# XiandaGuo/OpenStereo

Hardware: NVIDIA H100
Metric: stereo_pairs_per_sec_gwcnet_256x512_d192 (higher is better)
Workload: dtype f32

## Files before the change

### include/openstereo_b200.h

```cpp
#ifndef OPENSTEREO_B200_H_
#define OPENSTEREO_B200_H_

#include <stddef.h>
#include <stdint.h>

#ifdef __cplusplus
extern "C" {
#endif

#define OSB_OK 0
#define OSB_EINVAL 1
#define OSB_ECUDA 2
#define OSB_EUNSUPPORTED 3

#define OSB_ACT_NONE 0
#define OSB_ACT_RELU 1
#define OSB_ACT_LEAKY 2
#define OSB_ACT_RELU6 3
#define OSB_ACT_SIGMOID 4
#define OSB_ACT_TANH 5

typedef void* osb_stream_t;

int osb_abi_version(void);
const char* osb_last_error(void);
uint64_t osb_launch_count(void);
int osb_tc_overflow_count(osb_stream_t stream, int reset, unsigned int* count);
int osb_tc_overflow_poll(osb_stream_t stream, unsigned int* host_pinned);
const unsigned int* osb_tc_overflow_flag(void);
float osb_set_rz_kappa(float kappa);
int osb_set_persistent_grid_cap(int cap);
const char* osb_tc_last_variant(void);
const char* osb_volume_last_variant(void);


int osb_gwc_volume_fwd(const float* ref, const float* tgt, float* out, int B, int C, int H, int W,
                       int D, int G, osb_stream_t stream);

int osb_concat_volume_fwd(const float* ref, const float* tgt, float* out, int B, int C, int H,
                          int W, int D, int mask_left, osb_stream_t stream);

int osb_gwc_concat_volume_fwd(const float* ref_gwc, const float* tgt_gwc, const float* ref_cat,
                              const float* tgt_cat, float* out, int B, int Cg, int Cc, int H, int W,
                              int D, int G, osb_stream_t stream);

int osb_corr_volume_fwd(const float* left, const float* right, float* out, int B, int C, int H,
                        int W, int D, osb_stream_t stream);


int osb_softargmin_fwd(const float* cost, float* out, int B, int D, int H, int W, float alpha,
                       float start, float step, int normalize, osb_stream_t stream);

int osb_upsample_softargmin_fwd(const float* cost, float* out, int B, int Dl, int Hl, int Wl, int D,
                                int H, int W, int align_corners, osb_stream_t stream);

int osb_upsample_softargmin_values_fwd(const float* cost, const float* values, float* out, int B, int Dl, int Hl, int Wl,
                                       int D, int H, int W, int align_corners, osb_stream_t stream);

int osb_epe_partial_fwd(const float* pred, const float* gt, float* out, int B, int HW, float maxdisp,
                        osb_stream_t stream);


int osb_conv3d_k3_bn_act_fwd(const float* x, const float* w_packed, const float* scale,
                             const float* shift, const float* residual, const float* gate, float* y,
                             int B, int Cin, int Cout, int D, int H, int W, int stride, int act,
                             osb_stream_t stream);

// ... 114 lines not shown
```

### openstereo_b200/_lib.py

```python
import ctypes
import os

_PKG = os.path.dirname(os.path.abspath(__file__))
LIB_PATH = os.path.join(_PKG, "lib", "libopenstereo_b200.so")

_f32p = ctypes.c_void_p
_i = ctypes.c_int
_f = ctypes.c_float
_s = ctypes.c_void_p

SIGNATURES = {
    "osb_gwc_volume_fwd": [_f32p, _f32p, _f32p, _i, _i, _i, _i, _i, _i, _s],
    "osb_concat_volume_fwd": [_f32p, _f32p, _f32p, _i, _i, _i, _i, _i, _i, _s],
    "osb_gwc_concat_volume_fwd": [_f32p, _f32p, _f32p, _f32p, _f32p, _i, _i, _i, _i, _i, _i, _i, _s],
    "osb_corr_volume_fwd": [_f32p, _f32p, _f32p, _i, _i, _i, _i, _i, _s],
    "osb_softargmin_fwd": [_f32p, _f32p, _i, _i, _i, _i, _f, _f, _f, _i, _s],
    "osb_upsample_softargmin_fwd": [_f32p, _f32p, _i, _i, _i, _i, _i, _i, _i, _i, _s],
    "osb_epe_partial_fwd": [_f32p, _f32p, _f32p, _i, _i, _f, _s],
    "osb_conv3d_k3_bn_act_fwd": [_f32p] * 7 + [_i] * 8 + [_s],
    "osb_deconv3d_bn_act_fwd": [_f32p] * 6 + [_i] * 8 + [_s],
    "osb_conv3d_1x1_bn_act_fwd": [_f32p, _f32p, _i] + [_f32p] * 6 + [_i] * 8 + [_s],
    "osb_conv3d_tc_supported": [_i, _i, _i, _i],
    "osb_conv3d_tc_kc": [_i, _i, _i, _i],
    "osb_tc_general_width": [_i],
    "osb_conv3d_s2_tc_supported": [_i, _i, _i, _i, _i],
    "osb_deconv3d_tc_supported": [_i, _i, _i],
    "osb_deconv3d_k3_tc_fwd": [_f32p] * 6 + [_i] * 9 + [_s],
    "osb_conv3d_k3_s2_tc_fwd": [_f32p] * 6 + [_i] * 9 + [_s],
    "osb_conv3d_k3_tc_fwd": [_f32p] * 6 + [_i] * 9 + [_s],
    "osb_conv3d_k3_tc_ncdhw_fwd": [_f32p] * 6 + [_i] * 9 + [_s],
    "osb_conv3d_k3_tc_split_fwd": [_f32p] * 6 + [_i] * 10 + [_s],
    "osb_ncdhw_to_split": [_f32p, _f32p] + [_i] * 5 + [_s],
    "osb_conv3d_k3_tc_gate_fwd": [_f32p] * 7 + [_i] * 7 + [_s],
    "osb_deconv3d_k4_tc_supported": [_i, _i, _i],
    "osb_conv3d_k3_tc_cs_fwd": [_f32p] * 7 + [_i] * 8 + [_s],
    "osb_conv3d_k3_s2_tc_cs_fwd": [_f32p] * 5 + [_i] * 8 + [_s],
    "osb_deconv3d_k4_tc_cs_fwd": [_f32p] * 5 + [_i] * 8 + [_s],
# ... 87 lines not shown
```

### openstereo_b200/aggregation.py

```python
import torch

from . import ops
from .ops import ACT_LEAKY, ACT_NONE, ACT_RELU, ACT_RELU6


class _Packed:
    __slots__ = ("w", "scale", "shift", "stride", "kernel", "transposed", "cin", "cout", "_w5", "_tc")

    def __init__(self, conv, bn=None):
        self._tc = {}
        self._w5 = conv.weight.detach() if conv.weight.dim() == 5 else None
        self.cin, self.cout = (conv.in_channels, conv.out_channels)
        self.transposed = isinstance(conv, (torch.nn.ConvTranspose3d, torch.nn.ConvTranspose2d))
        self.kernel = int(conv.kernel_size[0])
        self.stride = int(conv.stride[0])
        self._validate(conv)
        wt = conv.weight
        if wt.dim() == 4:
            wt = wt.unsqueeze(2)
        if self.transposed:
            self.w = ops.pack_deconv_weight(wt)
        else:
            self.w = ops.pack_conv_weight(wt)
        if self.kernel == 1:
# ... 41 lines not shown
    kc = ops.conv3d_tc_kc(layer.cin, layer.cout, width)
    if not kc:
        return None
    if kc not in layer._tc:
        layer._tc[kc] = ops.pack_tc_weight(layer._w5, kc, pad_cout_to=16 if layer.cout < 16 else None)
    return layer._tc[kc]


def _tc_ok(layer, width):
    return _tc_weight(layer, width) is not None


def _conv_tc(layer, x_ndhwc, act=ACT_NONE, residual=None, out_ndhwc=True, res_ndhwc=True, in_ncdhw=False, out_split=False):
    wt = _tc_weight(layer, x_ndhwc.shape[4] if in_ncdhw else x_ndhwc.shape[3])
    return ops.conv3d_k3_tc(x_ndhwc, wt, layer.scale, layer.shift, residual, act, out_ndhwc, res_ndhwc, in_ncdhw,
                            out_split=out_split)


def _split_chain_ok(width, *layers):
    return USE_TENSOR_CORES and all(ops.conv3d_tc_kc(l.cin, l.cout, width) == 32 for l in layers)


def _stem_in(layer, volume, act, out_split=False):
    if ops.conv3d_tc_kc(layer.cin, layer.cout, volume.shape[-1]) == 32:
        return _conv_tc(layer, volume, act, in_ncdhw=True, out_split=out_split)
    return _conv_tc(layer, ops.to_ndhwc(volume), act)


def _conv_auto(layer, x, act=ACT_NONE, residual=None):
    if layer.stride == 1 and _tc_ok(layer, x.shape[-1]):
        return _conv_tc(layer, ops.to_ndhwc(x), act, residual, out_ndhwc=False, res_ndhwc=False)
    if (USE_TENSOR_CORES and layer.stride == 2 and layer.kernel == 3 and not layer.transposed and layer._w5 is not None
            and ops.conv3d_s2_tc_supported(layer.cin, layer.cout, x.shape[2], x.shape[3], x.shape[4])):
        if "s2" not in layer._tc:
            layer._tc["s2"] = ops.pack_tc_weight(layer._w5, 16, kw_order=(1, 0, 2))
        return ops.conv3d_k3_s2_tc(ops.to_ndhwc(x), layer._tc["s2"], layer.scale, layer.shift, residual, act)
    return _conv(layer, x, act, residual)


def _deconv(layer, x, act=ACT_NONE, residual=None):
    if (USE_TENSOR_CORES and layer.transposed and layer.kernel == 3 and layer._w5 is not None
            and ops.deconv3d_tc_supported(layer.cin, layer.cout, x.shape[-1])):
        if "dc" not in layer._tc:
            layer._tc["dc"] = ops.pack_tc_deconv_weight(layer._w5)
        return ops.deconv3d_k3_tc(ops.to_ndhwc(x), layer._tc["dc"], layer.scale, layer.shift, residual, act)
    return ops.deconv3d(x, layer.w, layer.scale, layer.shift, residual, layer.kernel, act)
# ... 88 lines not shown
    head0, cls = classif3
    width = out.shape[3]
    if _tc_ok(cls, width):
        mid = _conv_tc(head0, out, ACT_RELU, out_split=_split_chain_ok(width, head0, cls))
        return _conv_tc(cls, mid, ACT_NONE, out_ndhwc=False, res_ndhwc=False)
    if cls.cin == 32 and cls.cout == 1 and cls._w5 is not None and cls.stride == 1:
        if "c1" not in cls._tc:
            cls._tc["c1"] = ops.pack_c1_weight(cls._w5)
        head = _conv_tc(head0, out, ACT_RELU)
        return ops.conv3d_k3_c1_ndhwc(head, cls._tc["c1"], cls.scale, cls.shift)
    head = _conv_tc(head0, out, ACT_RELU, out_ndhwc=False)
    return _conv(cls, head)


class GwcAggregation(_Engine):

    def _pack(self):
        m = self.module
        self.dres0 = [_Packed(m.dres0[0][0], m.dres0[0][1]), _Packed(m.dres0[2][0], m.dres0[2][1])]
        self.dres1 = [_Packed(m.dres1[0][0], m.dres1[0][1]), _Packed(m.dres1[2][0], m.dres1[2][1])]
        self.hg = [_GwcHourglass(m.dres2), _GwcHourglass(m.dres3), _GwcHourglass(m.dres4)]
        self.classif3 = [_Packed(m.classif3[0][0], m.classif3[0][1]), _Packed(m.classif3[2])]

    def logits(self, volume):
        volume = self._check(volume)
        self._ensure(volume.device)
        width = volume.shape[-1]
        stem_tc = all(_tc_ok(l, width) for l in (self.dres0[0], self.dres0[1], self.dres1[0], self.dres1[1]))
        b, _, dd, hh, ww = volume.shape
        if stem_tc and _tc_ok(self.classif3[0], width) and all(_hg_channels_last_ok(hg, (b, dd, hh, ww, 32)) for hg in self.hg):
            split = _split_chain_ok(width, self.dres0[0], self.dres0[1], self.dres1[0], self.dres1[1])
            c = _conv_tc(self.dres0[1], _stem_in(self.dres0[0], volume, ACT_RELU, out_split=split), ACT_RELU, out_split=split)
            out = _conv_tc(self.dres1[1], _conv_tc(self.dres1[0], c, ACT_RELU, out_split=split), ACT_NONE, residual=c)
            for hg in self.hg:
                out = _gwc_hourglass_channels_last(hg, out)
            return _classif3_channels_last(self.classif3, out)
        if stem_tc:
            c = _conv_tc(self.dres0[1], _stem_in(self.dres0[0], volume, ACT_RELU), ACT_RELU)
            cost0 = _conv_tc(self.dres1[1], _conv_tc(self.dres1[0], c, ACT_RELU), ACT_NONE, residual=c, out_ndhwc=False)
        else:
            c = _conv(self.dres0[1], _conv(self.dres0[0], volume, ACT_RELU), ACT_RELU)
            cost0 = _conv(self.dres1[1], _conv(self.dres1[0], c, ACT_RELU), ACT_NONE, residual=c)
        out = cost0
        for hg in self.hg:
            out = hg(out)
        if _tc_ok(self.classif3[0], width):
            head = _conv_tc(self.classif3[0], ops.to_ndhwc(out), ACT_RELU, out_ndhwc=False)
        else:
            head = _conv(self.classif3[0], out, ACT_RELU)
        return _conv(self.classif3[1], head)

    def __call__(self, volume, h, w):
        mon = self._watch(volume.device)
        out = ops.upsample_softargmin(self.logits(volume), self.module.maxdisp, h, w, align_corners=False)
        if mon is not None:
            mon.poll()
        return out


class CascadeAggregation(GwcAggregation):

    def __call__(self, cost, fine_d, fine_h, fine_w, disp_range_samples):
        mon = self._watch(cost.device)
        assert tuple(disp_range_samples.shape[1:]) == (fine_d, fine_h, fine_w)
        out = ops.upsample_softargmin_values(self.logits(cost), disp_range_samples, align_corners=False)
        if mon is not None:
            mon.poll()
        return out


class _PSMHourglass:
    def __init__(self, m):
        self.conv1, self.conv2 = _Packed(m.conv1[0], m.conv1[1]), _Packed(m.conv2[0], m.conv2[1])
        self.conv3, self.conv4 = _Packed(m.conv3[0], m.conv3[1]), _Packed(m.conv4[0], m.conv4[1])
        self.conv5, self.conv6 = _Packed(m.conv5[0], m.conv5[1]), _Packed(m.conv6[0], m.conv6[1])

    def __call__(self, x, presqu, postsqu, skip):
# ... 630 lines not shown
```

### openstereo_b200/csrc/volume.cu

```cuda
#include <cstdlib>

#include "common.cuh"

namespace osb {

constexpr int kTileW = 128;
constexpr int kChunkD = 64;
constexpr int kRowW = kTileW + kChunkD;
constexpr int kJG = 4;

struct VolParams {
  const float* ref_g;
  const float* tgt_g;
  const float* ref_c;
  const float* tgt_c;
  float* out;
  int B, Cg, Cc, H, W, D, G, K;
  int Ctot, oc_cat;
  int GU, n_gwc_units, n_cat_units, w_tiles, d_chunks;
  int mask_left, use_tma, vec_ok;
  int order;
  float inv_k;
};

__device__ __forceinline__ float4 load_quad(const float* row, int w, int W, bool vec) {
  if (vec && w + 3 < W) return __ldg(reinterpret_cast<const float4*>(row + w));
  float4 v;
  v.x = (w + 0 < W) ? __ldg(row + w + 0) : 0.f;
  v.y = (w + 1 < W) ? __ldg(row + w + 1) : 0.f;
  v.z = (w + 2 < W) ? __ldg(row + w + 2) : 0.f;
  v.w = (w + 3 < W) ? __ldg(row + w + 3) : 0.f;
  return v;
}

__device__ __forceinline__ void store_quad(float* row, int w, int W, bool vec, float4 v) {
  if (vec && w + 3 < W) {
    st_cs_f4(row + w, v);
  } else {
    if (w + 0 < W) __stcs(row + w + 0, v.x);
    if (w + 1 < W) __stcs(row + w + 1, v.y);
    if (w + 2 < W) __stcs(row + w + 2, v.z);
    if (w + 3 < W) __stcs(row + w + 3, v.w);
  }
}

struct Item {
  int unit, h, b, w0, d0;
};
__device__ __forceinline__ Item decode_item(const VolParams& p, int it) {
  Item i;
  const int units = p.n_gwc_units + p.n_cat_units;
  if (p.order == 1) {
    i.h = it % p.H;
    it /= p.H;
    i.unit = it % units;
    it /= units;
  } else {
    i.unit = it % units;
    it /= units;
    i.h = it % p.H;
    it /= p.H;
  }
  i.d0 = (it % p.d_chunks) * kChunkD;
  it /= p.d_chunks;
  i.w0 = (it % p.w_tiles) * kTileW;
  i.b = it / p.w_tiles;
  return i;
}

template <bool VEC, bool K4>
__global__ void __launch_bounds__(256, 2) volume_kernel(const __grid_constant__ CUtensorMap tgt_map, const VolParams p,
                                                        const int total_items) {
  extern __shared__ __align__(128) float smem[];
  const int warp = threadIdx.x >> 5, lane = threadIdx.x & 31;
  const int rows = p.n_gwc_units > 0 ? p.GU * p.K : p.GU;
  const size_t buf_floats = (size_t)rows * kRowW;
  uint64_t* bars = reinterpret_cast<uint64_t*>(smem + 2 * buf_floats);
  const size_t HW = (size_t)p.H * p.W;
  constexpr bool vec = VEC;
  const uint32_t tx_bytes = (uint32_t)rows * kRowW * 4u;

  if (p.use_tma && threadIdx.x == 0) {
    tma_prefetch_desc(&tgt_map);
    mbar_init(&bars[0], 1);
    mbar_init(&bars[1], 1);
    fence_mbar_init();
  }
  __syncthreads();

  auto issue_tma = [&](int it, int stage) {
    const Item n = decode_item(p, it);
    if (n.unit < p.n_gwc_units) {
      fence_proxy_async();
      mbar_arrive_expect_tx(&bars[stage], tx_bytes);
      tma_load_3d(smem + stage * buf_floats, &tgt_map, &bars[stage], n.w0 - n.d0 - kChunkD, n.h,
                  n.b * p.Cg + n.unit * p.GU * p.K);
    }
  };

  int stage = 0;
  uint32_t phase0 = 0, phase1 = 0;
  if (p.use_tma && threadIdx.x == 0 && (int)blockIdx.x < total_items) issue_tma(blockIdx.x, 0);

// ... 10 lines not shown

    if (cur.unit < p.n_gwc_units) {
      const int g0 = cur.unit * p.GU;
      if (p.use_tma) {
        if (stage == 0) {
          mbar_wait(&bars[0], phase0);
          phase0 ^= 1;
        } else {
          mbar_wait(&bars[1], phase1);
          phase1 ^= 1;
        }
      } else {
        const int live = min(rows, p.Cg - g0 * p.K);
        for (int idx = threadIdx.x; idx < live * kRowW; idx += blockDim.x) {
          const int r = idx / kRowW, c = idx - r * kRowW;
          const int gw = col0 + c;
          float v = 0.f;
          if (gw >= 0 && gw < p.W) v = __ldg(p.tgt_g + ((size_t)(b * p.Cg + g0 * p.K + r) * p.H + h) * p.W + gw);
          buf[idx] = v;
        }
        __syncthreads();
      }
      const int g = g0 + warp;
      if (g < p.G && wq < p.W) {
        const float* lrow = p.ref_g + ((size_t)(b * p.Cg + g * p.K) * p.H + h) * p.W;
        const float* rbase = buf + (size_t)warp * p.K * kRowW;
        float* obase = p.out + (((size_t)(b * p.Ctot + g) * p.D) * p.H + h) * p.W;
        for (int j0 = 0; j0 < nquads; j0 += kJG) {
          float acc[kJG][4][4];
#pragma unroll
          for (int jj = 0; jj < kJG; ++jj)
#pragma unroll
            for (int i = 0; i < 4; ++i)
#pragma unroll
              for (int a = 0; a < 4; ++a) acc[jj][i][a] = 0.f;
          const int win = kChunkD + 4 * (lane - j0) - 16;
          for (int k0 = 0; k0 < p.K; k0 += 4) {
            float4 lq[4];
#pragma unroll
            for (int kk = 0; kk < 4; ++kk)
              lq[kk] = (K4 || k0 + kk < p.K) ? load_quad(lrow + (size_t)(k0 + kk) * HW, wq, p.W, vec) : make_float4(0.f, 0.f, 0.f, 0.f);
#pragma unroll
            for (int kk = 0; kk < 4; ++kk) {
              if (K4 || k0 + kk < p.K) {
                const float l[4] = {lq[kk].x * p.inv_k, lq[kk].y * p.inv_k, lq[kk].z * p.inv_k, lq[kk].w * p.inv_k};
                float r[20];
                const float4* rp = reinterpret_cast<const float4*>(rbase + (size_t)(k0 + kk) * kRowW + win);
#pragma unroll
                for (int n = 0; n < 5; ++n) {
                  const float4 t = rp[n];
                  r[4 * n + 0] = t.x, r[4 * n + 1] = t.y, r[4 * n + 2] = t.z, r[4 * n + 3] = t.w;
                }
#pragma unroll
                for (int jj = 0; jj < kJG; ++jj)
#pragma unroll
                  for (int i = 0; i < 4; ++i)
#pragma unroll
                    for (int a = 0; a < 4; ++a) acc[jj][i][a] = fmaf(l[a], r[16 - 4 * jj + a - i], acc[jj][i][a]);
              }
            }
          }
#pragma unroll
          for (int jj = 0; jj < kJG; ++jj) {
#pragma unroll
            for (int i = 0; i < 4; ++i) {
              const int d = d0 + 4 * (j0 + jj) + i;
              if (4 * (j0 + jj) + i < nd) {
                float4 v;
                v.x = (wq + 0 >= d) ? acc[jj][i][0] : 0.f;
                v.y = (wq + 1 >= d) ? acc[jj][i][1] : 0.f;
                v.z = (wq + 2 >= d) ? acc[jj][i][2] : 0.f;
                v.w = (wq + 3 >= d) ? acc[jj][i][3] : 0.f;
                store_quad(obase + (size_t)d * HW, wq, p.W, vec, v);
              }
            }
          }
        }
      }
    } else {
      const int oc = (cur.unit - p.n_gwc_units) * p.GU + warp;
      if (oc < 2 * p.Cc) {
        const bool left = oc < p.Cc;
        float* obase = p.out + (((size_t)(b * p.Ctot + p.oc_cat + oc) * p.D) * p.H + h) * p.W;
        if (left) {
          if (wq < p.W) {
            const float4 v = load_quad(p.ref_c + ((size_t)(b * p.Cc + oc) * p.H + h) * p.W, wq, p.W, vec);
            for (int dd = 0; dd < nd; ++dd) {
              const int d = d0 + dd;
              float4 o = v;
              if (p.mask_left) {
                o.x = (wq + 0 >= d) ? v.x : 0.f;
                o.y = (wq + 1 >= d) ? v.y : 0.f;
                o.z = (wq + 2 >= d) ? v.z : 0.f;
                o.w = (wq + 3 >= d) ? v.w : 0.f;
              }
              store_quad(obase + (size_t)d * HW, wq, p.W, vec, o);
            }
          }
        } else {
          float* row = buf + (size_t)warp * kRowW;
          const float* src = p.tgt_c + ((size_t)(b * p.Cc + (oc - p.Cc)) * p.H + h) * p.W;
          for (int c = lane; c < kRowW; c += 32) {
            const int gw = col0 + c;
            row[c] = (gw >= 0 && gw < p.W) ? __ldg(src + gw) : 0.f;
          }
          __syncwarp();
          if (wq < p.W) {
            for (int j = 0; j < nquads; ++j) {
              const float4 lo = *reinterpret_cast<const float4*>(row + kChunkD + 4 * (lane - j) - 4);
              const float4 hi = *reinterpret_cast<const float4*>(row + kChunkD + 4 * (lane - j));
              const float wv[8] = {lo.x, lo.y, lo.z, lo.w, hi.x, hi.y, hi.z, hi.w};
#pragma unroll
              for (int i = 0; i < 4; ++i) {
                const int d = d0 + 4 * j + i;
                if (4 * j + i < nd) {
                  float4 o;
                  o.x = wv[4 - i], o.y = wv[5 - i], o.z = wv[6 - i], o.w = wv[7 - i];
                  store_quad(obase + (size_t)d * HW, wq, p.W, vec, o);
                }
              }
            }
          }
        }
      }
    }
    __syncthreads();
  }
}

static thread_local const char* g_volume_variant = "";

static int launch_volume(const float* ref_g, const float* tgt_g, const float* ref_c, const float* tgt_c, float* out,
                         int B, int Cg, int Cc, int H, int W, int D, int G, int mask_left, cudaStream_t stream, int reduce_sum = 0) {
  OSB_REQUIRE(B > 0 && H > 0 && W > 0 && D > 0, "volume: empty shape B=%d H=%d W=%d D=%d", B, H, W, D);
  OSB_REQUIRE(Cg >= 0 && Cc >= 0 && (Cg > 0 || Cc > 0), "volume: no channels");
  int K = 0;
  if (Cg > 0) {
    OSB_REQUIRE(G > 0 && Cg % G == 0, "groupwise_correlation: C=%d not divisible by num_groups=%d", Cg, G);
    K = Cg / G;
    OSB_REQUIRE(K <= 144, "volume: %d channels per group exceeds the 144 supported (two-stage 192-float rows in 227 KB)", K);
  } else {
    G = 0;
  }
  VolParams p{};
  p.ref_g = ref_g, p.tgt_g = tgt_g, p.ref_c = ref_c, p.tgt_c = tgt_c, p.out = out;
  p.B = B, p.Cg = Cg, p.Cc = Cc, p.H = H, p.W = W, p.D = D, p.G = G, p.K = K;
  p.Ctot = G + 2 * Cc, p.oc_cat = G;
  int GU = 8;
  if (Cg > 0) {
    GU = G < 8 ? G : 8;
    while (GU > 1 && GU * K > 128) GU >>= 1;
  }
  p.GU = GU;
  p.n_gwc_units = Cg > 0 ? (G + GU - 1) / GU : 0;
  p.n_cat_units = Cc > 0 ? (2 * Cc + GU - 1) / GU : 0;
  p.w_tiles = (W + kTileW - 1) / kTileW;
  p.d_chunks = (D + kChunkD - 1) / kChunkD;
  p.mask_left = mask_left;
  {
    static const int order = [] {
      const char* e = getenv("OSB_VOLUME_ORDER");
      return e ? atoi(e) : 1;
    }();
    p.order = order;
  }
  p.inv_k = K > 0 ? (reduce_sum ? 1.0f : 1.0f / (float)K) : 0.f;
  auto aligned16 = [](const void* q) { return q == nullptr || (reinterpret_cast<uintptr_t>(q) & 15) == 0; };
  p.vec_ok = (W % 4 == 0) && aligned16(ref_g) && aligned16(ref_c) && aligned16(out);
  const int rows = Cg > 0 ? GU * K : GU;
  size_t smem = 2 * (size_t)rows * kRowW * sizeof(float) + 16;
  CUtensorMap map{};
  p.use_tma = 0;
  if (Cg > 0 && W % 4 == 0 && aligned16(tgt_g) && rows <= 256) {
    if (make_tensor_map_3d(&map, tgt_g, (uint64_t)W, (uint64_t)H, (uint64_t)B * Cg, (uint64_t)W * 4, (uint64_t)H * W * 4,
                           kRowW, 1, (uint32_t)rows))
      p.use_tma = 1;
  }
  using KernelFn = void (*)(const CUtensorMap, const VolParams, const int);
  const bool k4 = (K % 4 == 0);
  const int variant = (p.vec_ok ? 2 : 0) | (k4 ? 1 : 0);
  static const KernelFn kernels[4] = {volume_kernel<false, false>, volume_kernel<false, true>, volume_kernel<true, false>,
                                      volume_kernel<true, true>};
  KernelFn kernel = kernels[variant];
  static size_t configured_all[64][4] = {};
  size_t* configured = configured_all[device_index() & 63];
  if (smem > configured[variant]) {
    cudaError_t e = cudaFuncSetAttribute(kernel, cudaFuncAttributeMaxDynamicSharedMemorySize, (int)smem);
    if (e != cudaSuccess) {
      set_error("volume: cannot reserve %zu bytes of shared memory: %s", smem, cudaGetErrorString(e));
      return OSB_ECUDA;
    }
    configured[variant] = smem;
  }
  const long long total = (long long)(p.n_gwc_units + p.n_cat_units) * H * B * p.w_tiles * p.d_chunks;
  OSB_REQUIRE(total < (1ll << 31), "volume: too many work items (%lld)", total);
  static const char* const names[8] = {"volume<0,0,ldg>", "volume<0,0,tma>", "volume<0,1,ldg>", "volume<0,1,tma>",
                                       "volume<1,0,ldg>", "volume<1,0,tma>", "volume<1,1,ldg>", "volume<1,1,tma>"};
  g_volume_variant = names[2 * variant + p.use_tma];
  int per_sm = 0;
  cudaError_t oe = cudaOccupancyMaxActiveBlocksPerMultiprocessor(&per_sm, kernel, 32 * GU, smem);
  if (oe != cudaSuccess || per_sm < 1) {
    set_error("volume: occupancy query failed (%s), smem=%zu", cudaGetErrorString(oe), smem);
    (void)cudaGetLastError();
    return OSB_ECUDA;
  }
  long long grid = (long long)sm_count() * per_sm;
  if (grid > total) grid = total;
  grid = cap_persistent_grid(grid);
  kernel<<<(unsigned)grid, 32 * GU, smem, stream>>>(map, p, (int)total);
  count_launch();
  return check_launch("volume_kernel");
}

}

extern "C" {

const char* osb_volume_last_variant(void) { return osb::g_volume_variant; }

int osb_gwc_volume_fwd(const float* ref, const float* tgt, float* out, int B, int C, int H, int W, int D, int G,
                       osb_stream_t stream) {
  OSB_REQUIRE(ref && tgt && out, "gwc_volume: null pointer");
  OSB_REQUIRE(C > 0, "gwc_volume: C=%d", C);
  return osb::launch_volume(ref, tgt, nullptr, nullptr, out, B, C, 0, H, W, D, G, 1, (cudaStream_t)stream);
}

int osb_gwc_volume_sum_fwd(const float* ref, const float* tgt, float* out, int B, int C, int H, int W, int D, int G,
                           osb_stream_t stream) {
  OSB_REQUIRE(ref && tgt && out, "gwc_volume_sum: null pointer");
  OSB_REQUIRE(C > 0, "gwc_volume_sum: C=%d", C);
  return osb::launch_volume(ref, tgt, nullptr, nullptr, out, B, C, 0, H, W, D, G, 1, (cudaStream_t)stream, 1);
}

int osb_concat_volume_fwd(const float* ref, const float* tgt, float* out, int B, int C, int H, int W, int D,
                          int mask_left, osb_stream_t stream) {
  OSB_REQUIRE(ref && tgt && out, "concat_volume: null pointer");
  OSB_REQUIRE(C > 0, "concat_volume: C=%d", C);
  return osb::launch_volume(nullptr, nullptr, ref, tgt, out, B, 0, C, H, W, D, 0, mask_left, (cudaStream_t)stream);
}

int osb_gwc_concat_volume_fwd(const float* ref_gwc, const float* tgt_gwc, const float* ref_cat, const float* tgt_cat,
                              float* out, int B, int Cg, int Cc, int H, int W, int D, int G, osb_stream_t stream) {
  OSB_REQUIRE(ref_gwc && tgt_gwc && ref_cat && tgt_cat && out, "gwc_concat_volume: null pointer");
  OSB_REQUIRE(Cg > 0 && Cc > 0, "gwc_concat_volume: Cg=%d Cc=%d", Cg, Cc);
  return osb::launch_volume(ref_gwc, tgt_gwc, ref_cat, tgt_cat, out, B, Cg, Cc, H, W, D, G, 1, (cudaStream_t)stream);
}

int osb_corr_volume_fwd(const float* left, const float* right, float* out, int B, int C, int H, int W, int D,
                        osb_stream_t stream) {
  OSB_REQUIRE(left && right && out, "corr_volume: null pointer");
  OSB_REQUIRE(C > 0, "corr_volume: C=%d", C);
  return osb::launch_volume(left, right, nullptr, nullptr, out, B, C, 0, H, W, D, 1, 1, (cudaStream_t)stream);
}
}
```

### openstereo_b200/host_models.py

```python
import torch
import torch.nn as nn
import torch.nn.functional as F

from . import aggregation as _agg
from . import ops
from .aggregation import GwcAggregation, PSMAggregation


USE_TC_BACKBONE = True


def _cfg_get(cfgs, key, default=None):
    if isinstance(cfgs, dict):
        return cfgs.get(key, default)
    return getattr(cfgs, key, default)


def _cb(cin, cout, k, stride, pad, dilation, bias=False):
    return nn.Sequential(nn.Conv2d(cin, cout, kernel_size=k, stride=stride, padding=dilation if dilation > 1 else pad,
                                   dilation=dilation, bias=bias), nn.BatchNorm2d(cout))


def _front_tc_ok(net, x):
    return (getattr(net, "_osb_folded", False) and x.is_cuda and x.dim() == 4 and x.shape[2] == 2 * ops.TC_WIDTH and x.shape[3] % 2 == 0
# ... 295 lines not shown

def _db3(cin, cout):
    return nn.Sequential(nn.ConvTranspose3d(cin, cout, 3, padding=1, output_padding=1, stride=2, bias=False), nn.BatchNorm3d(cout))


class _GwcHourglassParams(nn.Module):
    def __init__(self, c):
        super().__init__()
        r = lambda: nn.ReLU(inplace=True)
        self.conv1 = nn.Sequential(_cb3(c, 2 * c, 3, 2, 1), r())
        self.conv2 = nn.Sequential(_cb3(2 * c, 2 * c, 3, 1, 1), r())
        self.conv3 = nn.Sequential(_cb3(2 * c, 4 * c, 3, 2, 1), r())
        self.conv4 = nn.Sequential(_cb3(4 * c, 4 * c, 3, 1, 1), r())
        self.conv5, self.conv6 = _db3(4 * c, 2 * c), _db3(2 * c, c)
        self.redir1, self.redir2 = _cb3(c, c, 1, 1, 0), _cb3(2 * c, 2 * c, 1, 1, 0)


class GwcVolumeCostProcessor(nn.Module):

    def __init__(self, maxdisp=192, downsample=4, num_groups=40, use_concat_volume=True, *args, **kwargs):
        super().__init__()
        self.maxdisp, self.downsample, self.num_groups, self.use_concat_volume = maxdisp, downsample, num_groups, use_concat_volume

    def forward(self, inputs):
        lf, rf = inputs["ref_feature"], inputs["tgt_feature"]
        d = self.maxdisp // self.downsample
        if self.use_concat_volume:
            vol = ops.gwc_concat_volume(lf["gwc_feature"], rf["gwc_feature"], lf["concat_feature"], rf["concat_feature"],
                                        d, self.num_groups)
        else:
            vol = ops.build_gwc_volume(lf["gwc_feature"], rf["gwc_feature"], d, self.num_groups)
        return {"cost_volume": vol}


class GwcDispProcessor(nn.Module):

    def __init__(self, maxdisp=192, downsample=4, num_groups=40, use_concat_volume=True, concat_channels=12, *args, **kwargs):
        super().__init__()
        self.maxdisp = maxdisp
        cin = num_groups + (2 * concat_channels if use_concat_volume else 0)
        r = lambda: nn.ReLU(inplace=True)
        self.dres0 = nn.Sequential(_cb3(cin, 32, 3, 1, 1), r(), _cb3(32, 32, 3, 1, 1), r())
        self.dres1 = nn.Sequential(_cb3(32, 32, 3, 1, 1), r(), _cb3(32, 32, 3, 1, 1))
        self.dres2, self.dres3, self.dres4 = _GwcHourglassParams(32), _GwcHourglassParams(32), _GwcHourglassParams(32)
        for i in range(4):
            setattr(self, "classif%d" % i, nn.Sequential(_cb3(32, 32, 3, 1, 1), r(),
                                                         nn.Conv3d(32, 1, kernel_size=3, padding=1, stride=1, bias=False)))
        self._engine = None

    def forward(self, inputs):
        if self.training:
            raise RuntimeError("openstereo_b200.GwcDispProcessor implements the inference branch only (model.eval())")
        if self._engine is None:
            self._engine = GwcAggregation(self)
        h, w = inputs["left"].shape[2:]
        return {"inference_disp": {"disp_est": self._engine(inputs["cost_volume"], h, w)}}


class GwcNet(nn.Module):
    def __init__(self, cfgs):
        super().__init__()
        self.maxdisp = _cfg_get(cfgs, "MAX_DISP", 192)
        use_concat, cc = _cfg_get(cfgs, "USE_CONCAT_VOLUME", True), _cfg_get(cfgs, "CONCAT_CHANNELS", 12)
        ds, g = _cfg_get(cfgs, "DOWNSAMPLE", 4), _cfg_get(cfgs, "NUM_GROUPS", 40)
        self.Backbone = _GwcBackbone(use_concat, cc if use_concat else 0)
        self.CostProcessor = GwcVolumeCostProcessor(self.maxdisp, ds, g, use_concat)
        self.DispProcessor = GwcDispProcessor(self.maxdisp, ds, g, use_concat, cc)

    def forward(self, inputs):
        inputs.update(self.Backbone(inputs))
        inputs.update(self.CostProcessor(inputs))
        return {"disp_pred": self.DispProcessor(inputs)["inference_disp"]["disp_est"]}


def _cbr3(cin, cout, k=3, s=1, p=1):
    return nn.Sequential(nn.Conv3d(cin, cout, kernel_size=k, stride=s, padding=p, dilation=1, bias=False),
                         nn.BatchNorm3d(cout), nn.ReLU(inplace=True))


class _PsmHourglassParams(nn.Module):
    def __init__(self, c):
        super().__init__()
        self.conv1, self.conv2 = _cbr3(c, 2 * c, 3, 2, 1), _cb3(2 * c, 2 * c, 3, 1, 1)
        self.conv3, self.conv4 = _cbr3(2 * c, 2 * c, 3, 2, 1), _cbr3(2 * c, 2 * c, 3, 1, 1)
        self.conv5, self.conv6 = _db3(2 * c, 2 * c), _db3(2 * c, c)


class _PsmAggregatorParams(nn.Module):
    def __init__(self, max_disp, in_planes=64):
        super().__init__()
        self.max_disp = max_disp
        self.dres0 = nn.Sequential(_cbr3(in_planes, 32), _cbr3(32, 32))
        self.dres1 = nn.Sequential(_cbr3(32, 32), _cb3(32, 32, 3, 1, 1))
        self.dres2, self.dres3, self.dres4 = _PsmHourglassParams(32), _PsmHourglassParams(32), _PsmHourglassParams(32)
        for i in (1, 2, 3):
# ... 52 lines not shown
```

### openstereo_b200/ops.py

```python
import math

import torch

from . import _lib

ACT_NONE, ACT_RELU, ACT_LEAKY, ACT_RELU6 = 0, 1, 2, 3
TC_WIDTH = 128
TC_KC = 32


_LAUNCH_DEVICE = [None]


def _stream(t):
    _LAUNCH_DEVICE[0] = t.device.index
    return torch.cuda.current_stream(t.device).cuda_stream


def _same_device(*tensors):
    devs = {t.device for t in tensors if t is not None}
    if len(devs) > 1:
        raise RuntimeError("openstereo_b200: operands live on different devices: %s" % sorted(str(d) for d in devs))


# ... 140 lines not shown
    ys, _ = _prep(y, "y")
    assert xs.dim() == 4 and xs.shape == ys.shape
    _same_device(xs, ys)
    b, c, h, w = xs.shape
    assert c % group == 0
    out = torch.empty((b, group, maxdisp + 1, h, w), dtype=torch.float32, device=xs.device)
    if out.numel():
        _call("osb_gwc_volume_sum_fwd", xs.data_ptr(), ys.data_ptr(), out.data_ptr(), b, c, h, w, maxdisp + 1, group, _stream(out))
    return out.to(dt)


def build_sub_volume(feat_l, feat_r, maxdisp):
    l, dt = _prep(feat_l, "feat_l")
    r, _ = _prep(feat_r, "feat_r")
    assert l.dim() == 4 and l.shape == r.shape
    _same_device(l, r)
    b, c, h, w = l.shape
    out = torch.empty((b, maxdisp, h, w), dtype=torch.float32, device=l.device)
    if out.numel():
        _call("osb_sub_volume_fwd", l.data_ptr(), r.data_ptr(), out.data_ptr(), b, c, h, w, maxdisp, _stream(out))
    return out.to(dt)


def gwc_concat_volume(ref_gwc, tgt_gwc, ref_cat, tgt_cat, maxdisp, num_groups):
    rg, dt = _prep(ref_gwc, "ref_gwc")
    tg, _ = _prep(tgt_gwc, "tgt_gwc")
    rc, _ = _prep(ref_cat, "ref_cat")
    tc, _ = _prep(tgt_cat, "tgt_cat")
    assert rg.shape == tg.shape and rc.shape == tc.shape and rg.shape[0] == rc.shape[0] and rg.shape[2:] == rc.shape[2:]
    _same_device(rg, tg, rc, tc)
    b, cg, h, w = rg.shape
    cc = rc.shape[1]
    assert cg % num_groups == 0
    out = torch.empty((b, num_groups + 2 * cc, maxdisp, h, w), dtype=torch.float32, device=rg.device)
    if out.numel():
        _call("osb_gwc_concat_volume_fwd", rg.data_ptr(), tg.data_ptr(), rc.data_ptr(), tc.data_ptr(),
                  out.data_ptr(), b, cg, cc, h, w, maxdisp, num_groups, _stream(out))
    return out.to(dt)


def _no_autograd(name, *tensors):
    if _recording(*tensors):
        raise RuntimeError("openstereo_b200.ops.%s has no backward: call it under torch.no_grad() or on operands that do not "
                           "require grad" % name)


def warped_concat_volume(x, y, disp_samples, mask_left=False):
    _no_autograd("warped_concat_volume", x, y, disp_samples)
    xs, dt = _prep(x, "x")
    ys, _ = _prep(y, "y")
    ds, _ = _prep(disp_samples, "disp_samples")
    assert xs.dim() == 4 and xs.shape == ys.shape and ds.dim() == 4
    b, c, h, w = xs.shape
    assert ds.shape[0] == b and ds.shape[2:] == (h, w)
    _same_device(xs, ys, ds)
    d = ds.shape[1]
    out = torch.empty((b, 2 * c, d, h, w), dtype=torch.float32, device=xs.device)
    if out.numel():
        _call("osb_warped_concat_volume_fwd", xs.data_ptr(), ys.data_ptr(), ds.data_ptr(), out.data_ptr(), b, c, d, h, w,
              1 if mask_left else 0, _stream(out))
    return out.to(dt)
# ... 770 lines not shown
```

Measured before the change: 313.3.

## Emit GwcNet cost volume directly in split fp16 channels-last layout

The gwc+concat volume kernel gains a split output mode that writes the volume as hi/lo fp16 pairs in a channels-last (B,D,H,W,2C) layout. It stages each tile in shared memory and exchanges halves across a 2-CTA cluster so each thread issues wide streaming stores. GwcNet now routes this layout straight into the first tensor-core conv when supported. This removes the separate fp32 NCDHW volume write and the conversion pass the stem conv needed. The cost is cluster syncs per d-quad, extra shared memory and an fp16 overflow check, and the split path drops the per-thread bounds checks.

```diff
diff --git a/include/openstereo_b200.h b/include/openstereo_b200.h
--- a/include/openstereo_b200.h
+++ b/include/openstereo_b200.h
@@ -43,6 +43,11 @@
 int osb_gwc_concat_volume_fwd(const float* ref_gwc, const float* tgt_gwc, const float* ref_cat,
                               const float* tgt_cat, float* out, int B, int Cg, int Cc, int H, int W,
                               int D, int G, osb_stream_t stream);
+
+int osb_gwc_concat_volume_split_supported(int Cg, int Cc, int G);
+int osb_gwc_concat_volume_split_fwd(const float* ref_gwc, const float* tgt_gwc, const float* ref_cat,
+                                    const float* tgt_cat, float* out_split, int B, int Cg, int Cc, int H,
+                                    int W, int D, int G, osb_stream_t stream);
 
 int osb_corr_volume_fwd(const float* left, const float* right, float* out, int B, int C, int H,
                         int W, int D, osb_stream_t stream);
diff --git a/openstereo_b200/_lib.py b/openstereo_b200/_lib.py
--- a/openstereo_b200/_lib.py
+++ b/openstereo_b200/_lib.py
@@ -13,6 +13,8 @@
     "osb_gwc_volume_fwd": [_f32p, _f32p, _f32p, _i, _i, _i, _i, _i, _i, _s],
     "osb_concat_volume_fwd": [_f32p, _f32p, _f32p, _i, _i, _i, _i, _i, _i, _s],
     "osb_gwc_concat_volume_fwd": [_f32p, _f32p, _f32p, _f32p, _f32p, _i, _i, _i, _i, _i, _i, _i, _s],
+    "osb_gwc_concat_volume_split_supported": [_i, _i, _i],
+    "osb_gwc_concat_volume_split_fwd": [_f32p, _f32p, _f32p, _f32p, _f32p, _i, _i, _i, _i, _i, _i, _i, _s],
     "osb_corr_volume_fwd": [_f32p, _f32p, _f32p, _i, _i, _i, _i, _i, _s],
     "osb_softargmin_fwd": [_f32p, _f32p, _i, _i, _i, _i, _f, _f, _f, _i, _s],
     "osb_upsample_softargmin_fwd": [_f32p, _f32p, _i, _i, _i, _i, _i, _i, _i, _i, _s],
diff --git a/openstereo_b200/aggregation.py b/openstereo_b200/aggregation.py
--- a/openstereo_b200/aggregation.py
+++ b/openstereo_b200/aggregation.py
@@ -87,6 +87,8 @@
 
 
 def _stem_in(layer, volume, act, out_split=False):
+    if ops.is_split(volume):
+        return _conv_tc(layer, volume, act, out_split=out_split)
     if ops.conv3d_tc_kc(layer.cin, layer.cout, volume.shape[-1]) == 32:
         return _conv_tc(layer, volume, act, in_ncdhw=True, out_split=out_split)
     return _conv_tc(layer, ops.to_ndhwc(volume), act)
@@ -221,20 +223,38 @@
         self.hg = [_GwcHourglass(m.dres2), _GwcHourglass(m.dres3), _GwcHourglass(m.dres4)]
         self.classif3 = [_Packed(m.classif3[0][0], m.classif3[0][1]), _Packed(m.classif3[2])]
 
-    def logits(self, volume):
-        volume = self._check(volume)
-        self._ensure(volume.device)
-        width = volume.shape[-1]
-        stem_tc = all(_tc_ok(l, width) for l in (self.dres0[0], self.dres0[1], self.dres1[0], self.dres1[1]))
-        b, _, dd, hh, ww = volume.shape
-        if stem_tc and _tc_ok(self.classif3[0], width) and all(_hg_channels_last_ok(hg, (b, dd, hh, ww, 32)) for hg in self.hg):
-            split = _split_chain_ok(width, self.dres0[0], self.dres0[1], self.dres1[0], self.dres1[1])
-            c = _conv_tc(self.dres0[1], _stem_in(self.dres0[0], volume, ACT_RELU, out_split=split), ACT_RELU, out_split=split)
-            out = _conv_tc(self.dres1[1], _conv_tc(self.dres1[0], c, ACT_RELU, out_split=split), ACT_NONE, residual=c)
+    def _channels_last_ok(self, b, d, h, w):
+        stem = (self.dres0[0], self.dres0[1], self.dres1[0], self.dres1[1])
+        return (all(_tc_ok(l, w) for l in stem) and _tc_ok(self.classif3[0], w)
+                and all(_hg_channels_last_ok(hg, (b, d, h, w, 32)) for hg in self.hg))
+
+    def split_volume_ok(self, shape, device):
+        b, c, d, h, w = shape
+        if device.type != "cuda" or c % 32:
+            return False
+        self._ensure(device)
+        return self._channels_last_ok(b, d, h, w) and _split_chain_ok(w, self.dres0[0])
+
+    def logits(self, volume, split=False):
+        if split:
+            if not ops.is_split(volume):
+                raise ValueError("GwcAggregation: split=True needs a split (B, D, H, W, 2C) fp16 volume")
+            b, dd, hh, ww, c2 = volume.shape
+            if not self.split_volume_ok((b, c2 // 2, dd, hh, ww), volume.device):
+                raise ValueError("GwcAggregation: no split-input route for a volume of shape %s" % (tuple(volume.shape),))
+        else:
+            volume = self._check(volume)
+            self._ensure(volume.device)
+            b, _, dd, hh, ww = volume.shape
+        width = ww
+        if self._channels_last_ok(b, dd, hh, ww):
+            chain = _split_chain_ok(width, self.dres0[0], self.dres0[1], self.dres1[0], self.dres1[1])
+            c = _conv_tc(self.dres0[1], _stem_in(self.dres0[0], volume, ACT_RELU, out_split=chain), ACT_RELU, out_split=chain)
+            out = _conv_tc(self.dres1[1], _conv_tc(self.dres1[0], c, ACT_RELU, out_split=chain), ACT_NONE, residual=c)
             for hg in self.hg:
                 out = _gwc_hourglass_channels_last(hg, out)
             return _classif3_channels_last(self.classif3, out)
-        if stem_tc:
+        if all(_tc_ok(l, width) for l in (self.dres0[0], self.dres0[1], self.dres1[0], self.dres1[1])):
             c = _conv_tc(self.dres0[1], _stem_in(self.dres0[0], volume, ACT_RELU), ACT_RELU)
             cost0 = _conv_tc(self.dres1[1], _conv_tc(self.dres1[0], c, ACT_RELU), ACT_NONE, residual=c, out_ndhwc=False)
         else:
@@ -249,9 +269,9 @@
             head = _conv(self.classif3[0], out, ACT_RELU)
         return _conv(self.classif3[1], head)
 
-    def __call__(self, volume, h, w):
+    def __call__(self, volume, h, w, split=False):
         mon = self._watch(volume.device)
-        out = ops.upsample_softargmin(self.logits(volume), self.module.maxdisp, h, w, align_corners=False)
+        out = ops.upsample_softargmin(self.logits(volume, split), self.module.maxdisp, h, w, align_corners=False)
         if mon is not None:
             mon.poll()
         return out
diff --git a/openstereo_b200/csrc/volume.cu b/openstereo_b200/csrc/volume.cu
--- a/openstereo_b200/csrc/volume.cu
+++ b/openstereo_b200/csrc/volume.cu
@@ -1,6 +1,7 @@
+#include <cooperative_groups.h>
 #include <cstdlib>
 
-#include "common.cuh"
+#include "tc_common.cuh"
 
 namespace osb {
 
@@ -8,6 +9,8 @@
 constexpr int kChunkD = 64;
 constexpr int kRowW = kTileW + kChunkD;
 constexpr int kJG = 4;
+constexpr int kSplitGU = 8;
+constexpr size_t kSplitStageBytes = 4 * kSplitGU * 2 * kTileW * sizeof(uint16_t);
 
 struct VolParams {
   const float* ref_g;
@@ -15,6 +18,8 @@
   const float* ref_c;
   const float* tgt_c;
   float* out;
+  uint16_t* out_split;
+  unsigned int* overflow;
   int B, Cg, Cc, H, W, D, G, K;
   int Ctot, oc_cat;
   int GU, n_gwc_units, n_cat_units, w_tiles, d_chunks;
@@ -50,7 +55,14 @@
 __device__ __forceinline__ Item decode_item(const VolParams& p, int it) {
   Item i;
   const int units = p.n_gwc_units + p.n_cat_units;
-  if (p.order == 1) {
+  if (p.order == 2) {
+    const int pair = it & 1;
+    it >>= 1;
+    i.h = it % p.H;
+    it /= p.H;
+    i.unit = 2 * (it % (units / 2)) + pair;
+    it /= units / 2;
+  } else if (p.order == 1) {
     i.h = it % p.H;
     it /= p.H;
     i.unit = it % units;
@@ -78,7 +90,36 @@
   uint64_t* bars = reinterpret_cast<uint64_t*>(smem + 2 * buf_floats);
   const size_t HW = (size_t)p.H * p.W;
   constexpr bool vec = VEC;
+  const bool split = VEC && p.out_split != nullptr;
   const uint32_t tx_bytes = (uint32_t)rows * kRowW * 4u;
+  uint16_t* stage_h = reinterpret_cast<uint16_t*>(bars + 2);
+  float amax = 0.f;
+  auto split_stage = [&](int i, float4 v) {
+    uint2 hi, lo;
+    f16_split4(v, hi, lo, amax);
+    uint16_t* s = stage_h + ((i * kSplitGU + (threadIdx.x >> 5)) * 2) * kTileW + 4 * (threadIdx.x & 31);
+    *reinterpret_cast<uint2*>(s) = hi;
+    *reinterpret_cast<uint2*>(s + kTileW) = lo;
+  };
+  auto split_flush = [&](int c0, int d0, int dl, int nd, int b, int h, int w0) {
+    cooperative_groups::cluster_group cluster = cooperative_groups::this_cluster();
+    cluster.sync();
+    const int m = threadIdx.x & 3;
+    const int wl = (int)cluster.block_rank() * (kTileW / 2) + (threadIdx.x >> 2);
+    const uint16_t* src = cluster.map_shared_rank(stage_h, m & 1);
+    if (w0 + wl < p.W) {
+#pragma unroll 1
+      for (int i = 0; i < 4 && dl + i < nd; ++i) {
+        const uint16_t* s = src + (i * kSplitGU * 2 + (m >> 1)) * kTileW + wl;
+        uint32_t q[4];
+#pragma unroll
+        for (int c = 0; c < 4; ++c) q[c] = (uint32_t)s[(2 * c) * 2 * kTileW] | ((uint32_t)s[(2 * c + 1) * 2 * kTileW] << 16);
+        uint16_t* vox = p.out_split + ((((size_t)b * p.D + d0 + dl + i) * p.H + h) * p.W + w0 + wl) * 2 * p.Ctot;
+        __stcs(reinterpret_cast<uint4*>(vox + split_index(c0 & ~(SPLIT_GRANULE - 1)) + m * kSplitGU), make_uint4(q[0], q[1], q[2], q[3]));
+      }
+    }
+    cluster.sync();
+  };
 
   if (p.use_tma && threadIdx.x == 0) {
     tma_prefetch_desc(&tgt_map);
@@ -135,7 +176,7 @@
         __syncthreads();
       }
       const int g = g0 + warp;
-      if (g < p.G && wq < p.W) {
+      if (split || (g < p.G && wq < p.W)) {
         const float* lrow = p.ref_g + ((size_t)(b * p.Cg + g * p.K) * p.H + h) * p.W;
         const float* rbase = buf + (size_t)warp * p.K * kRowW;
         float* obase = p.out + (((size_t)(b * p.Ctot + g) * p.D) * p.H + h) * p.W;
@@ -178,36 +219,46 @@
 #pragma unroll
             for (int i = 0; i < 4; ++i) {
               const int d = d0 + 4 * (j0 + jj) + i;
-              if (4 * (j0 + jj) + i < nd) {
+              if (split || 4 * (j0 + jj) + i < nd) {
                 float4 v;
                 v.x = (wq + 0 >= d) ? acc[jj][i][0] : 0.f;
                 v.y = (wq + 1 >= d) ? acc[jj][i][1] : 0.f;
                 v.z = (wq + 2 >= d) ? acc[jj][i][2] : 0.f;
                 v.w = (wq + 3 >= d) ? acc[jj][i][3] : 0.f;
-                store_quad(obase + (size_t)d * HW, wq, p.W, vec, v);
+                if (split) split_stage(i, v);
+                else store_quad(obase + (size_t)d * HW, wq, p.W, vec, v);
               }
             }
+            if (split && 4 * (j0 + jj) < nd) split_flush(g0, d0, 4 * (j0 + jj), nd, b, h, w0);
           }
         }
       }
     } else {
       const int oc = (cur.unit - p.n_gwc_units) * p.GU + warp;
-      if (oc < 2 * p.Cc) {
+      const int c0 = p.oc_cat + (cur.unit - p.n_gwc_units) * p.GU;
+      if (split || oc < 2 * p.Cc) {
         const bool left = oc < p.Cc;
         float* obase = p.out + (((size_t)(b * p.Ctot + p.oc_cat + oc) * p.D) * p.H + h) * p.W;
         if (left) {
-          if (wq < p.W) {
+          if (split || wq < p.W) {
             const float4 v = load_quad(p.ref_c + ((size_t)(b * p.Cc + oc) * p.H + h) * p.W, wq, p.W, vec);
-            for (int dd = 0; dd < nd; ++dd) {
-              const int d = d0 + dd;
-              float4 o = v;
-              if (p.mask_left) {
-                o.x = (wq + 0 >= d) ? v.x : 0.f;
-                o.y = (wq + 1 >= d) ? v.y : 0.f;
-                o.z = (wq + 2 >= d) ? v.z : 0.f;
-                o.w = (wq + 3 >= d) ? v.w : 0.f;
+            for (int j = 0; j < nquads; ++j) {
+#pragma unroll
+              for (int i = 0; i < 4; ++i) {
+                const int d = d0 + 4 * j + i;
+                if (split || 4 * j + i < nd) {
+                  float4 o = v;
+                  if (p.mask_left) {
+                    o.x = (wq + 0 >= d) ? v.x : 0.f;
+                    o.y = (wq + 1 >= d) ? v.y : 0.f;
+                    o.z = (wq + 2 >= d) ? v.z : 0.f;
+                    o.w = (wq + 3 >= d) ? v.w : 0.f;
+                  }
+                  if (split) split_stage(i, o);
+                  else store_quad(obase + (size_t)d * HW, wq, p.W, vec, o);
+                }
               }
-              store_quad(obase + (size_t)d * HW, wq, p.W, vec, o);
+              if (split) split_flush(c0, d0, 4 * j, nd, b, h, w0);
             }
           }
         } else {
@@ -218,7 +269,7 @@
             row[c] = (gw >= 0 && gw < p.W) ? __ldg(src + gw) : 0.f;
           }
           __syncwarp();
-          if (wq < p.W) {
+          if (split || wq < p.W) {
             for (int j = 0; j < nquads; ++j) {
               const float4 lo = *reinterpret_cast<const float4*>(row + kChunkD + 4 * (lane - j) - 4);
               const float4 hi = *reinterpret_cast<const float4*>(row + kChunkD + 4 * (lane - j));
@@ -226,12 +277,14 @@
 #pragma unroll
               for (int i = 0; i < 4; ++i) {
                 const int d = d0 + 4 * j + i;
-                if (4 * j + i < nd) {
+                if (split || 4 * j + i < nd) {
                   float4 o;
                   o.x = wv[4 - i], o.y = wv[5 - i], o.z = wv[6 - i], o.w = wv[7 - i];
-                  store_quad(obase + (size_t)d * HW, wq, p.W, vec, o);
+                  if (split) split_stage(i, o);
+                  else store_quad(obase + (size_t)d * HW, wq, p.W, vec, o);
                 }
               }
+              if (split) split_flush(c0, d0, 4 * j, nd, b, h, w0);
             }
           }
         }
@@ -239,12 +292,19 @@
     }
     __syncthreads();
   }
+  if (split) tc_report_overflow(p.overflow, amax);
 }
 
 static thread_local const char* g_volume_variant = "";
 
+static bool split_volume_supported(int Cg, int Cc, int G) {
+  return Cg > 0 && Cc > 0 && G > 0 && Cg % G == 0 && Cg / G <= 128 / kSplitGU && G % kSplitGU == 0 && Cc % 4 == 0 &&
+         (G + 2 * Cc) % 32 == 0;
+}
+
 static int launch_volume(const float* ref_g, const float* tgt_g, const float* ref_c, const float* tgt_c, float* out,
-                         int B, int Cg, int Cc, int H, int W, int D, int G, int mask_left, cudaStream_t stream, int reduce_sum = 0) {
+                         int B, int Cg, int Cc, int H, int W, int D, int G, int mask_left, cudaStream_t stream, int reduce_sum = 0,
+                         uint16_t* out_split = nullptr) {
   OSB_REQUIRE(B > 0 && H > 0 && W > 0 && D > 0, "volume: empty shape B=%d H=%d W=%d D=%d", B, H, W, D);
   OSB_REQUIRE(Cg >= 0 && Cc >= 0 && (Cg > 0 || Cc > 0), "volume: no channels");
   int K = 0;
@@ -256,7 +316,7 @@
     G = 0;
   }
   VolParams p{};
-  p.ref_g = ref_g, p.tgt_g = tgt_g, p.ref_c = ref_c, p.tgt_c = tgt_c, p.out = out;
+  p.ref_g = ref_g, p.tgt_g = tgt_g, p.ref_c = ref_c, p.tgt_c = tgt_c, p.out = out, p.out_split = out_split;
   p.B = B, p.Cg = Cg, p.Cc = Cc, p.H = H, p.W = W, p.D = D, p.G = G, p.K = K;
   p.Ctot = G + 2 * Cc, p.oc_cat = G;
   int GU = 8;
@@ -265,6 +325,14 @@
     while (GU > 1 && GU * K > 128) GU >>= 1;
   }
   p.GU = GU;
+  const bool split = out_split != nullptr;
+  if (split) {
+    OSB_REQUIRE(split_volume_supported(Cg, Cc, G) && GU == kSplitGU,
+                "gwc_concat_volume_split: Cg=%d Cc=%d G=%d: needs a concat part, G a multiple of %d with at most %d channels per "
+                "group, Cc a multiple of 4 and G + 2*Cc a multiple of 32", Cg, Cc, G, kSplitGU, 128 / kSplitGU);
+    p.overflow = tc_overflow_flag();
+    if (!p.overflow) return OSB_ECUDA;
+  }
   p.n_gwc_units = Cg > 0 ? (G + GU - 1) / GU : 0;
   p.n_cat_units = Cc > 0 ? (2 * Cc + GU - 1) / GU : 0;
   p.w_tiles = (W + kTileW - 1) / kTileW;
@@ -275,13 +343,16 @@
       const char* e = getenv("OSB_VOLUME_ORDER");
       return e ? atoi(e) : 1;
     }();
-    p.order = order;
+    p.order = out_split ? 2 : order;
   }
   p.inv_k = K > 0 ? (reduce_sum ? 1.0f : 1.0f / (float)K) : 0.f;
   auto aligned16 = [](const void* q) { return q == nullptr || (reinterpret_cast<uintptr_t>(q) & 15) == 0; };
   p.vec_ok = (W % 4 == 0) && aligned16(ref_g) && aligned16(ref_c) && aligned16(out);
+  OSB_REQUIRE(!split || (p.vec_ok && aligned16(out_split)),
+              "gwc_concat_volume_split: W=%d must be a multiple of 4 and every tensor 16-byte aligned", W);
   const int rows = Cg > 0 ? GU * K : GU;
   size_t smem = 2 * (size_t)rows * kRowW * sizeof(float) + 16;
+  if (split) smem += kSplitStageBytes;
   CUtensorMap map{};
   p.use_tma = 0;
   if (Cg > 0 && W % 4 == 0 && aligned16(tgt_g) && rows <= 256) {
@@ -307,9 +378,12 @@
   }
   const long long total = (long long)(p.n_gwc_units + p.n_cat_units) * H * B * p.w_tiles * p.d_chunks;
   OSB_REQUIRE(total < (1ll << 31), "volume: too many work items (%lld)", total);
-  static const char* const names[8] = {"volume<0,0,ldg>", "volume<0,0,tma>", "volume<0,1,ldg>", "volume<0,1,tma>",
-                                       "volume<1,0,ldg>", "volume<1,0,tma>", "volume<1,1,ldg>", "volume<1,1,tma>"};
-  g_volume_variant = names[2 * variant + p.use_tma];
+  static const char* const names[16] = {"volume<0,0,ldg>", "volume<0,0,tma>", "volume<0,1,ldg>", "volume<0,1,tma>",
+                                        "volume<1,0,ldg>", "volume<1,0,tma>", "volume<1,1,ldg>", "volume<1,1,tma>",
+                                        "volume<0,0,ldg,split>", "volume<0,0,tma,split>", "volume<0,1,ldg,split>",
+                                        "volume<0,1,tma,split>", "volume<1,0,ldg,split>", "volume<1,0,tma,split>",
+                                        "volume<1,1,ldg,split>", "volume<1,1,tma,split>"};
+  g_volume_variant = names[(split ? 8 : 0) + 2 * variant + p.use_tma];
   int per_sm = 0;
   cudaError_t oe = cudaOccupancyMaxActiveBlocksPerMultiprocessor(&per_sm, kernel, 32 * GU, smem);
   if (oe != cudaSuccess || per_sm < 1) {
@@ -320,7 +394,25 @@
   long long grid = (long long)sm_count() * per_sm;
   if (grid > total) grid = total;
   grid = cap_persistent_grid(grid);
-  kernel<<<(unsigned)grid, 32 * GU, smem, stream>>>(map, p, (int)total);
+  if (split) {
+    grid = grid >= 2 ? grid & ~1ll : 2;
+    cudaLaunchConfig_t cfg = {};
+    cfg.gridDim = dim3((unsigned)grid);
+    cfg.blockDim = dim3(32 * GU);
+    cfg.dynamicSmemBytes = smem;
+    cfg.stream = stream;
+    cudaLaunchAttribute attr[1];
+    attr[0].id = cudaLaunchAttributeClusterDimension;
+    attr[0].val.clusterDim.x = 2, attr[0].val.clusterDim.y = 1, attr[0].val.clusterDim.z = 1;
+    cfg.attrs = attr, cfg.numAttrs = 1;
+    const cudaError_t le = cudaLaunchKernelEx(&cfg, kernel, map, p, (int)total);
+    if (le != cudaSuccess) {
+      set_error("volume: cluster launch failed: %s", cudaGetErrorString(le));
+      return OSB_ECUDA;
+    }
+  } else {
+    kernel<<<(unsigned)grid, 32 * GU, smem, stream>>>(map, p, (int)total);
+  }
   count_launch();
   return check_launch("volume_kernel");
 }
@@ -359,6 +451,15 @@
   return osb::launch_volume(ref_gwc, tgt_gwc, ref_cat, tgt_cat, out, B, Cg, Cc, H, W, D, G, 1, (cudaStream_t)stream);
 }
 
+int osb_gwc_concat_volume_split_supported(int Cg, int Cc, int G) { return osb::split_volume_supported(Cg, Cc, G) ? 1 : 0; }
+
+int osb_gwc_concat_volume_split_fwd(const float* ref_gwc, const float* tgt_gwc, const float* ref_cat, const float* tgt_cat,
+                                    float* out_split, int B, int Cg, int Cc, int H, int W, int D, int G, osb_stream_t stream) {
+  OSB_REQUIRE(ref_gwc && tgt_gwc && ref_cat && tgt_cat && out_split, "gwc_concat_volume_split: null pointer");
+  return osb::launch_volume(ref_gwc, tgt_gwc, ref_cat, tgt_cat, nullptr, B, Cg, Cc, H, W, D, G, 1, (cudaStream_t)stream, 0,
+                            reinterpret_cast<uint16_t*>(out_split));
+}
+
 int osb_corr_volume_fwd(const float* left, const float* right, float* out, int B, int C, int H, int W, int D,
                         osb_stream_t stream) {
   OSB_REQUIRE(left && right && out, "corr_volume: null pointer");
diff --git a/openstereo_b200/host_models.py b/openstereo_b200/host_models.py
--- a/openstereo_b200/host_models.py
+++ b/openstereo_b200/host_models.py
@@ -341,12 +341,12 @@
         super().__init__()
         self.maxdisp, self.downsample, self.num_groups, self.use_concat_volume = maxdisp, downsample, num_groups, use_concat_volume
 
-    def forward(self, inputs):
+    def forward(self, inputs, out_split=False):
         lf, rf = inputs["ref_feature"], inputs["tgt_feature"]
         d = self.maxdisp // self.downsample
         if self.use_concat_volume:
             vol = ops.gwc_concat_volume(lf["gwc_feature"], rf["gwc_feature"], lf["concat_feature"], rf["concat_feature"],
-                                        d, self.num_groups)
+                                        d, self.num_groups, out_split=out_split)
         else:
             vol = ops.build_gwc_volume(lf["gwc_feature"], rf["gwc_feature"], d, self.num_groups)
         return {"cost_volume": vol}
@@ -367,13 +367,16 @@
                                                          nn.Conv3d(32, 1, kernel_size=3, padding=1, stride=1, bias=False)))
         self._engine = None
 
-    def forward(self, inputs):
+    def engine(self):
+        if self._engine is None:
+            self._engine = GwcAggregation(self)
+        return self._engine
+
+    def forward(self, inputs, split_volume=False):
         if self.training:
             raise RuntimeError("openstereo_b200.GwcDispProcessor implements the inference branch only (model.eval())")
-        if self._engine is None:
-            self._engine = GwcAggregation(self)
         h, w = inputs["left"].shape[2:]
-        return {"inference_disp": {"disp_est": self._engine(inputs["cost_volume"], h, w)}}
+        return {"inference_disp": {"disp_est": self.engine()(inputs["cost_volume"], h, w, split=split_volume)}}
 
 
 class GwcNet(nn.Module):
@@ -388,8 +391,20 @@
 
     def forward(self, inputs):
         inputs.update(self.Backbone(inputs))
-        inputs.update(self.CostProcessor(inputs))
-        return {"disp_pred": self.DispProcessor(inputs)["inference_disp"]["disp_est"]}
+        split = self._split_volume(inputs)
+        inputs.update(self.CostProcessor(inputs, out_split=split))
+        return {"disp_pred": self.DispProcessor(inputs, split_volume=split)["inference_disp"]["disp_est"]}
+
+    def _split_volume(self, inputs):
+        cp = self.CostProcessor
+        if not cp.use_concat_volume or self.DispProcessor.training:
+            return False
+        fg, fc = inputs["ref_feature"]["gwc_feature"], inputs["ref_feature"]["concat_feature"]
+        b, cg, h, w = fg.shape
+        cc = fc.shape[1]
+        shape = (b, cp.num_groups + 2 * cc, cp.maxdisp // cp.downsample, h, w)
+        return (ops.gwc_concat_volume_split_supported(cg, cc, cp.num_groups)
+                and self.DispProcessor.engine().split_volume_ok(shape, fg.device))
 
 
 def _cbr3(cin, cout, k=3, s=1, p=1):
diff --git a/openstereo_b200/ops.py b/openstereo_b200/ops.py
--- a/openstereo_b200/ops.py
+++ b/openstereo_b200/ops.py
@@ -186,7 +186,7 @@
     return out.to(dt)
 
 
-def gwc_concat_volume(ref_gwc, tgt_gwc, ref_cat, tgt_cat, maxdisp, num_groups):
+def gwc_concat_volume(ref_gwc, tgt_gwc, ref_cat, tgt_cat, maxdisp, num_groups, out_split=False):
     rg, dt = _prep(ref_gwc, "ref_gwc")
     tg, _ = _prep(tgt_gwc, "tgt_gwc")
     rc, _ = _prep(ref_cat, "ref_cat")
@@ -196,11 +196,20 @@
     b, cg, h, w = rg.shape
     cc = rc.shape[1]
     assert cg % num_groups == 0
+    if out_split:
+        out = torch.empty((b, maxdisp, h, w, 2 * (num_groups + 2 * cc)), dtype=torch.float16, device=rg.device)
+        _call("osb_gwc_concat_volume_split_fwd", rg.data_ptr(), tg.data_ptr(), rc.data_ptr(), tc.data_ptr(),
+              out.data_ptr(), b, cg, cc, h, w, maxdisp, num_groups, _stream(out), profile_as="osb_gwc_concat_volume_fwd")
+        return out
     out = torch.empty((b, num_groups + 2 * cc, maxdisp, h, w), dtype=torch.float32, device=rg.device)
     if out.numel():
         _call("osb_gwc_concat_volume_fwd", rg.data_ptr(), tg.data_ptr(), rc.data_ptr(), tc.data_ptr(),
                   out.data_ptr(), b, cg, cc, h, w, maxdisp, num_groups, _stream(out))
     return out.to(dt)
+
+
+def gwc_concat_volume_split_supported(cg, cc, num_groups):
+    return bool(_lib.lib.osb_gwc_concat_volume_split_supported(int(cg), int(cc), int(num_groups)))
 
 
 def _no_autograd(name, *tensors):
```

Measured after the change: 320.7, median of 6. 1.02x the previous value.
